# tzt101/MichiGAN

Measured on AMD Instinct MI355X. Metric: training images/sec at 512x512 (G+D step), higher is better.
Workload: dtype bf16; 1 GPU; SPADEB G + multiscale PatchGAN D + VGG19 + Gabor orientation losses, full G step + D step (Adam), bs=8/GPU, 512x512, BASELINE.json configs[2]; global_batch=8, batch_per_gpu=8, resolution=512, parallelism=dp1, init=reference default (xavier, 0.02), random VGG weights

## Files before the change

michigan_amd/csrc/mg_wgrad.hip:

```cpp
#include "mg_common.h"
#include "mg_wgrad_common.h"
#include "mg_options.h"



namespace {

constexpr int NTHR = 256;

struct WgK {
    const void* x; const void* dy; float* dw; float* dbias;
    int N, Hin, Win, Cin, Hj, Wj, Cg, isy, isx, ntaps;
    int K;
    int kper;
    int tiles_m, tiles_n, splitk;
    int tpt;
    long det_stride;
    int tap[MG_MAX_TAPS];
};

template <typename T, bool TR>
__global__ __launch_bounds__(NTHR) void wgrad_kernel(const WgK d)
{
    constexpr bool BF = (sizeof(T) == 2);
    constexpr int KP  = BF ? 32 : 16;
    constexpr int EPP = 16 / (int)sizeof(T);
    constexpr int PPR = 128 * (int)sizeof(T) / 16;
    constexpr int RPP = NTHR / PPR;
    constexpr int NPASS = KP / RPP;
    constexpr int RS  = BF ? 320 : 528;
    constexpr int OPB = KP * RS;
    constexpr int STAGE = 2 * OPB;

    extern __shared__ __attribute__((aligned(16))) unsigned char smem[];

    const int tid = threadIdx.x, lane = tid & 63, wave = tid >> 6;
    const int wm = wave >> 1, wn = wave & 1;
    const int l31 = lane & 31, hi = lane >> 5;

    int tile;
    {
        const int nblk = gridDim.x, b = blockIdx.x;
        const int q8 = nblk >> 3, r8 = nblk & 7, xcd = b & 7, idx = b >> 3;
        tile = (xcd < r8 ? xcd * (q8 + 1) : r8 * (q8 + 1) + (xcd - r8) * q8) + idx;
    }
    const int ngroups = (d.ntaps + d.tpt - 1) / d.tpt;
    const int tm = tile % d.tiles_m;  tile /= d.tiles_m;
    const int tn = tile % d.tiles_n;  tile /= d.tiles_n;
    const int tg = tile % ngroups;
    const int split = tile / ngroups;
    const int m0 = tm * 128, n0 = tn * 128;
    const int tap0 = tg * d.tpt;
    const int kbeg = split * d.kper;
    const int kend = min(d.K, kbeg + d.kper);
    if (kbeg >= kend) return;


    const T* __restrict__ X  = reinterpret_cast<const T*>(d.x);
    const T* __restrict__ DY = reinterpret_cast<const T*>(d.dy);
    const int HWj = d.Hj * d.Wj;

    const int piece = tid % PPR, prow = tid / PPR;
    const int ca = m0 + piece * EPP;
    const bool cav = ca < d.Cg;
    int mytap, cb;
    if (d.tpt > 1) { const int e = piece * EPP; mytap = tap0 + e / d.Cin; cb = e % d.Cin; }
    else           { mytap = tap0; cb = n0 + piece * EPP; }
    const bool cbv = (mytap < d.ntaps) && (cb < d.Cin);
    const int tp = d.tap[mytap < d.ntaps ? mytap : 0];
    const int tdy = (int)(short)(tp & 0xffff), tdx = tp >> 16;

    uint4 ra[NPASS], rb[NPASS];
    auto gload = [&](int k0) {
#pragma unroll
        for (int i = 0; i < NPASS; ++i) {
            const int q = k0 + prow + i * RPP;
            uint4 va = make_uint4(0, 0, 0, 0), vb = make_uint4(0, 0, 0, 0);
            if (q < kend) {
                if (cav) va = *reinterpret_cast<const uint4*>(DY + ((size_t)q * d.Cg + ca));
                if (cbv) {
                    const int n = q / HWj, r = q - n * HWj;
                    const int jy = r / d.Wj, jx = r - jy * d.Wj;
                    const int iy = jy * d.isy + tdy, ix = jx * d.isx + tdx;
                    if ((unsigned)iy < (unsigned)d.Hin && (unsigned)ix < (unsigned)d.Win)
                        vb = *reinterpret_cast<const uint4*>(X + ((size_t)((n * d.Hin + iy) * d.Win + ix) * d.Cin + cb));
                }
            }
            ra[i] = va; rb[i] = vb;
        }
    };
    auto lstore = [&](int s) {
        unsigned char* base = smem + s * STAGE;
#pragma unroll
        for (int i = 0; i < NPASS; ++i) {
            const int row = prow + i * RPP;
            *reinterpret_cast<uint4*>(base + row * RS + piece * 16) = ra[i];
            *reinterpret_cast<uint4*>(base + OPB + row * RS + piece * 16) = rb[i];
        }
    };

    f32x16_t acc[2][2];
#pragma unroll
    for (int mt = 0; mt < 2; ++mt)
#pragma unroll
        for (int nt = 0; nt < 2; ++nt)
#pragma unroll
            for (int r = 0; r < 16; ++r) acc[mt][nt][r] = 0.f;

    const bool do_bias = d.dbias != nullptr && tg == 0 && tn == 0;
    float bsum[EPP];
#pragma unroll
    for (int j = 0; j < EPP; ++j) bsum[j] = 0.f;
    auto bias_acc = [&]() {
#pragma unroll
        for (int i = 0; i < NPASS; ++i) {
            const uint32_t w[4] = {ra[i].x, ra[i].y, ra[i].z, ra[i].w};
            if constexpr (BF) {
#pragma unroll
                for (int j = 0; j < 4; ++j) { bsum[2 * j] += __uint_as_float(w[j] << 16); bsum[2 * j + 1] += __uint_as_float(w[j] & 0xffff0000u); }
            } else {
#pragma unroll
                for (int j = 0; j < 4; ++j) bsum[j] += __uint_as_float(w[j]);
            }
        }
    };

    auto compute = [&](int s) {
        const unsigned char* As = smem + s * STAGE;
        const unsigned char* Bs = As + OPB;
        if constexpr (BF) {
#pragma unroll
            for (int ks = 0; ks < 2; ++ks) {
                bf16x8_t a[2], b[2];
                if constexpr (TR) {
                    const int i16 = lane & 15, g2 = lane >> 4;
                    const int row = ks * 16 + (g2 >> 1) * 8 + (i16 >> 2);
                    const int col = (g2 & 1) * 16 + (i16 & 3) * 4;
#pragma unroll
                    for (int t = 0; t < 2; ++t) {
                        typedef __attribute__((address_space(3))) s16x4_t* lp_t;
                        const unsigned char* pa = As + row * RS + (wm * 64 + t * 32 + col) * 2;
                        const unsigned char* pb = Bs + row * RS + (wn * 64 + t * 32 + col) * 2;
                        s16x4_t a0 = __builtin_amdgcn_ds_read_tr16_b64_v4i16((lp_t)(pa));
                        s16x4_t a1 = __builtin_amdgcn_ds_read_tr16_b64_v4i16((lp_t)(pa + 4 * RS));
                        s16x4_t b0 = __builtin_amdgcn_ds_read_tr16_b64_v4i16((lp_t)(pb));
                        s16x4_t b1 = __builtin_amdgcn_ds_read_tr16_b64_v4i16((lp_t)(pb + 4 * RS));
                        typedef __attribute__((ext_vector_type(8))) short s16x8_t;
                        s16x8_t av = __builtin_shufflevector(a0, a1, 0, 1, 2, 3, 4, 5, 6, 7);
                        s16x8_t bv = __builtin_shufflevector(b0, b1, 0, 1, 2, 3, 4, 5, 6, 7);
                        a[t] = __builtin_bit_cast(bf16x8_t, av);
                        b[t] = __builtin_bit_cast(bf16x8_t, bv);
                    }
                } else {
                    typedef __attribute__((ext_vector_type(8))) short s16x8_t;
#pragma unroll
                    for (int t = 0; t < 2; ++t) {
                        s16x8_t av, bv;
#pragma unroll
                        for (int j = 0; j < 8; ++j) {
                            const int row = ks * 16 + hi * 8 + j;
                            av[j] = *reinterpret_cast<const short*>(As + row * RS + (wm * 64 + t * 32 + l31) * 2);
                            bv[j] = *reinterpret_cast<const short*>(Bs + row * RS + (wn * 64 + t * 32 + l31) * 2);
                        }
                        a[t] = __builtin_bit_cast(bf16x8_t, av);
                        b[t] = __builtin_bit_cast(bf16x8_t, bv);
                    }
                }
#pragma unroll
                for (int mt = 0; mt < 2; ++mt)
#pragma unroll
                    for (int nt = 0; nt < 2; ++nt)
                        acc[mt][nt] = __builtin_amdgcn_mfma_f32_32x32x16_bf16(a[mt], b[nt], acc[mt][nt], 0, 0, 0);
            }
        } else {
            f32x16_t t[2][2];
#pragma unroll
            for (int kk = 0; kk < KP / 2; ++kk) {
                float a[2], b[2];
                const int row = kk * 2 + hi;
#pragma unroll
                for (int q = 0; q < 2; ++q) {
                    a[q] = *reinterpret_cast<const float*>(As + row * RS + (wm * 64 + q * 32 + l31) * 4);
                    b[q] = *reinterpret_cast<const float*>(Bs + row * RS + (wn * 64 + q * 32 + l31) * 4);
                }
#pragma unroll
                for (int mt = 0; mt < 2; ++mt)
#pragma unroll
                    for (int nt = 0; nt < 2; ++nt) {
                        f32x16_t c;
                        if (MG_F32_ONE_CHAIN) {
                            acc[mt][nt] = __builtin_amdgcn_mfma_f32_32x32x2f32(a[mt], b[nt], acc[mt][nt], 0, 0, 0);
                            continue;
                        }
                        if (kk == 0) {
#pragma unroll
                            for (int e = 0; e < 16; ++e) c[e] = 0.f;
                        } else {
                            c = t[mt][nt];
                        }
                        t[mt][nt] = __builtin_amdgcn_mfma_f32_32x32x2f32(a[mt], b[nt], c, 0, 0, 0);
                    }
            }
#pragma unroll
            for (int mt = 0; mt < 2; ++mt)
#pragma unroll
                for (int nt = 0; nt < 2; ++nt) {
                    if (MG_F32_ONE_CHAIN) continue;
                    acc[mt][nt] += t[mt][nt];
                    asm volatile("" : "+v"(acc[mt][nt]));
                }
        }
    };

    const int nk = (kend - kbeg + KP - 1) / KP;
    gload(kbeg);
    if (do_bias) bias_acc();
    lstore(0);
    __syncthreads();
    for (int it = 0; it < nk; ++it) {
        const bool more = (it + 1 < nk);
        if (more) gload(kbeg + (it + 1) * KP);
        compute(it & 1);
        if (more) { if (do_bias) bias_acc(); lstore((it + 1) & 1); }
        __syncthreads();
    }
    if (do_bias) {
        float* red = reinterpret_cast<float*>(smem);
#pragma unroll
        for (int j = 0; j < EPP; ++j) red[prow * 128 + piece * EPP + j] = bsum[j];
        __syncthreads();
        if (tid < 128 && m0 + tid < d.Cg) {
            float t = 0.f;
            for (int r = 0; r < RPP; ++r) t += red[r * 128 + tid];
            wg_accum(d.dbias, d.det_stride, split, (size_t)(m0 + tid), t);
        }
    }

#pragma unroll
    for (int mt = 0; mt < 2; ++mt)
#pragma unroll
        for (int nt = 0; nt < 2; ++nt) {
            const int nn = wn * 64 + nt * 32 + l31;
            int tap, ci;
            if (d.tpt > 1) { tap = tap0 + nn / d.Cin; ci = nn % d.Cin; }
            else           { tap = tap0; ci = n0 + nn; }
            if (tap >= d.ntaps || ci >= d.Cin) continue;
#pragma unroll
            for (int r = 0; r < 16; ++r) {
                const int co = m0 + wm * 64 + mt * 32 + (r & 3) + 8 * (r >> 2) + 4 * hi;
                if (co < d.Cg)
                    wg_accum(d.dw, d.det_stride, split, (size_t)(tap * d.Cg + co) * d.Cin + ci, acc[mt][nt][r]);
            }
        }
}

__global__ __launch_bounds__(256) void wgrad_det_finish_kernel(const float* __restrict__ ws, int nsplit, long stride, float* __restrict__ dw, long ndw,
                                                               float* __restrict__ dbias, int nbias)
{
    __shared__ float red[256];
    const long total = ndw + nbias;
    const int cl = threadIdx.x & 31, row = threadIdx.x >> 5;
    for (long i0 = blockIdx.x * 32L; i0 < total; i0 += gridDim.x * 32L) {
        const long i = i0 + cl;
        float a = 0.f;
        if (i < total) {
            const float* p = ws + i;
            int sp = row;
            for (; sp + 24 < nsplit; sp += 32) {
                const float v0 = p[(size_t)sp * stride], v1 = p[(size_t)(sp + 8) * stride], v2 = p[(size_t)(sp + 16) * stride], v3 = p[(size_t)(sp + 24) * stride];
                a += v0; a += v1; a += v2; a += v3;
            }
            for (; sp < nsplit; sp += 8) a += p[(size_t)sp * stride];
        }
        __syncthreads();
        red[threadIdx.x] = a;
        __syncthreads();
        if (row == 0 && i < total) {
#pragma unroll
            for (int r = 1; r < 8; ++r) a += red[r * 32 + cl];
            if (i < ndw) dw[i] += a; else dbias[i - ndw] += a;
        }
    }
}

template <typename T, bool TR>
int launch_wgrad(WgK& k, hipStream_t st, int* nsplit = nullptr, bool dry = false)
{
    constexpr bool BF = (sizeof(T) == 2);
    constexpr int KP = BF ? 32 : 16;
    constexpr int RS = BF ? 320 : 528;
    k.tiles_m = (k.Cg + 127) / 128;
    k.tpt = (k.Cin < 128 && 128 % k.Cin == 0) ? 128 / k.Cin : 1;
    k.tiles_n = k.tpt > 1 ? 1 : (k.Cin + 127) / 128;
    const long base = (long)k.tiles_m * k.tiles_n * ((k.ntaps + k.tpt - 1) / k.tpt);
    int S = k.splitk;
    if (S <= 0) {
        S = (int)((1536 + base - 1) / base);
        const int min_stages = mg_opt(MG_OPT_WGRAD_MIN_STAGES);
        int maxS = (k.K + KP * min_stages - 1) / (KP * min_stages);
        if (base * maxS < 256) {
            const int fill = (int)((256 + base - 1) / base), floor4 = (k.K + KP * 4 - 1) / (KP * 4);
            maxS = fill < floor4 ? fill : floor4;
        }
        if (S > maxS) S = maxS;
        if (S < 1) S = 1;
    }
    k.kper = ((k.K + S - 1) / S + KP - 1) / KP * KP;
    S = (k.K + k.kper - 1) / k.kper;
    k.splitk = S;
    const long nblk = base * S;
    if (nsplit) *nsplit = S;
    if (dry) return MG_OK;
    if (nblk <= 0 || nblk > 0x7fffffffL) return mg_fail(MG_ERR_ARG, "mg_conv_wgrad: bad grid %ld", nblk);
    const size_t lds = 2 * 2 * (size_t)KP * RS;
    hipLaunchKernelGGL((wgrad_kernel<T, TR>), dim3((unsigned)nblk), dim3(NTHR), lds, st, k);
    MG_CHECK_LAUNCH("mg_conv_wgrad");
    return MG_OK;
}

}

int launch_wgrad_det_finish(const float* ws, int nsplit, long stride, float* dw, long ndw, float* dbias, int nbias, hipStream_t st)
{
    const long total = ndw + nbias;
    long grid = (total + 31) / 32;
    if (grid > 8192) grid = 8192;
    hipLaunchKernelGGL(wgrad_det_finish_kernel, dim3((unsigned)grid), dim3(256), 0, st, ws, nsplit, stride, dw, ndw, dbias, nbias);
    MG_CHECK_LAUNCH("mg_conv_wgrad(deterministic finish)");
    return MG_OK;
}

namespace {

int route_wgrad(const mg_wgrad_desc* d, hipStream_t st, float* dw, float* dbias, long det_stride, int* nsplit, bool dry)
{
    WgK k;
    k.x = d->x; k.dy = d->dy; k.dw = dw; k.dbias = dbias;
    k.N = d->N; k.Hin = d->Hin; k.Win = d->Win; k.Cin = d->Cin;
    k.Hj = d->Hj; k.Wj = d->Wj; k.Cg = d->Cg; k.isy = d->isy; k.isx = d->isx; k.ntaps = d->ntaps;
    k.K = d->N * d->Hj * d->Wj; k.splitk = d->splitk; k.kper = 0; k.tiles_m = k.tiles_n = 0; k.tpt = 1; k.det_stride = det_stride;
    for (int t = 0; t < MG_MAX_TAPS; ++t)
        k.tap[t] = t < d->ntaps ? (int)((((uint32_t)(int)d->tap_dy[t]) & 0xffffu) | (((uint32_t)(int)d->tap_dx[t]) << 16)) : 0;
    if (d->dtype == MG_BF16 && d->ntaps == 9 && d->isy == 1 && d->isx == 1 && d->Hin == d->Hj && d->Win == d->Wj && d->Cin == 8) {
        bool std3x3 = true;
        for (int t = 0; t < 9; ++t) std3x3 = std3x3 && d->tap_dy[t] == t / 3 - 1 && d->tap_dx[t] == t % 3 - 1;
        Wg3K k3;
        k3.x = d->x; k3.dy = d->dy; k3.dw = dw; k3.dbias = dbias;
        k3.N = d->N; k3.H = d->Hin; k3.W = d->Win; k3.Cin = d->Cin; k3.Cg = d->Cg;
        k3.nstg = 0; k3.sps = 0; k3.tiles_m = k3.tiles_n = 0; k3.splitk = 0; k3.det_stride = det_stride; k3.half_cu = 0; k3.stripe_w = 0;
        if (std3x3 && wgrad_thin_applies(k3)) return launch_wgrad_thin(k3, st, nsplit, dry);
    }
    if (wgrad_thin_taps_applies(d)) return launch_wgrad_thin_taps(d, st, dw, dbias, det_stride, nsplit, dry);
    if (mg_opt(MG_OPT_WGRAD3X3) && d->dtype == MG_BF16 && (d->flags & 1) && d->ntaps == 9 && d->isy == 1 && d->isx == 1 &&
        d->Hin == d->Hj && d->Win == d->Wj && (d->Win == 16 || d->Win % 32 == 0) && (d->Hin * d->Win) % 32 == 0 &&
        d->Cin >= 64 && d->Cg >= 64) {
        bool std3x3 = true;
        for (int t = 0; t < 9; ++t) std3x3 = std3x3 && d->tap_dy[t] == t / 3 - 1 && d->tap_dx[t] == t % 3 - 1;
        if (std3x3) {
            Wg3K k3;
            k3.x = d->x; k3.dy = d->dy; k3.dw = dw; k3.dbias = dbias;
            k3.N = d->N; k3.H = d->Hin; k3.W = d->Win; k3.Cin = d->Cin; k3.Cg = d->Cg;
            k3.nstg = k.K / 32; k3.sps = 0; k3.tiles_m = k3.tiles_n = 0; k3.splitk = d->splitk; k3.det_stride = det_stride;
            k3.half_cu = (d->flags & 2) ? 1 : 0; k3.stripe_w = 0;
            return launch_wgrad3x3(k3, st, nsplit, dry);
        }
    }
    if (d->dtype == MG_BF16)
        return (d->flags & 1) ? launch_wgrad<uint16_t, true>(k, st, nsplit, dry) : launch_wgrad<uint16_t, false>(k, st, nsplit, dry);
    return launch_wgrad<float, false>(k, st, nsplit, dry);
}

int check_wgrad_desc(const mg_wgrad_desc* d, const char* who)
{
    MG_CHECK_ARG(d != nullptr, "%s: null descriptor", who);
    MG_CHECK_ARG(d->x && d->dy && d->dw, "%s: null tensor pointer", who);
    MG_CHECK_ARG(d->dtype == MG_F32 || d->dtype == MG_BF16, "%s: bad dtype %d", who, d->dtype);
    MG_CHECK_ARG(d->ntaps >= 1 && d->ntaps <= MG_MAX_TAPS, "%s: ntaps=%d out of range", who, d->ntaps);
    MG_CHECK_ARG(d->Cin > 0 && (d->Cin % 8) == 0 && d->Cg > 0 && (d->Cg % 8) == 0,
                 "%s: Cin=%d / Cg=%d must be positive multiples of 8", who, d->Cin, d->Cg);
    MG_CHECK_ARG(d->N > 0 && d->Hj > 0 && d->Wj > 0 && d->Hin > 0 && d->Win > 0, "%s: empty geometry", who);
    MG_CHECK_ARG((long)d->N * d->Hj * d->Wj < (1L << 30), "%s: too many pixels", who);
    return MG_OK;
}

}

extern "C" int64_t mg_wgrad_det_workspace(const mg_wgrad_desc* d)
{
    if (check_wgrad_desc(d, "mg_wgrad_det_workspace") != MG_OK) return -1;
    int S = 0;
    if (route_wgrad(d, nullptr, d->dw, d->dbias, 0, &S, true) != MG_OK || S <= 0) return -1;
    const long slab = (long)d->ntaps * d->Cg * d->Cin + (d->dbias ? d->Cg : 0);
    return (int64_t)S * slab * (int64_t)sizeof(float);
}

extern "C" int mg_conv_wgrad(const mg_wgrad_desc* d, void* stream)
{
    const int rc = check_wgrad_desc(d, "mg_conv_wgrad");
    if (rc != MG_OK) return rc;
    hipStream_t st = reinterpret_cast<hipStream_t>(stream);
    if (d->det_ws == nullptr) return route_wgrad(d, st, d->dw, d->dbias, 0, nullptr, false);
    int S = 0;
    if (route_wgrad(d, st, d->dw, d->dbias, 0, &S, true) != MG_OK || S <= 0) return mg_fail(MG_ERR_ARG, "mg_conv_wgrad: cannot size the deterministic workspace");
    const long ndw = (long)d->ntaps * d->Cg * d->Cin, nbias = d->dbias ? d->Cg : 0, slab = ndw + nbias;
    MG_CHECK_ARG(d->det_ws_bytes >= (int64_t)S * slab * (int64_t)sizeof(float), "mg_conv_wgrad: deterministic workspace too small (%ld splits)", (long)S);
    float* ws = reinterpret_cast<float*>(d->det_ws);
    int S2 = 0;
    const int r2 = route_wgrad(d, st, ws, d->dbias ? ws + ndw : nullptr, slab, &S2, false);
    if (r2 != MG_OK) return r2;
    if (S2 != S) return mg_fail(MG_ERR_LAUNCH, "mg_conv_wgrad: split count changed between sizing and launch (%d vs %d)", S, S2);
    return launch_wgrad_det_finish(ws, S, slab, d->dw, ndw, d->dbias, (int)nbias, st);
}
```

michigan_amd/csrc/mg_wgrad3x3.hip:

```cpp
#include "mg_conv_common.h"
#include "mg_wgrad_common.h"


namespace {

typedef __attribute__((ext_vector_type(4))) short s16x4_t;
typedef __attribute__((ext_vector_type(8))) short s16x8_t;
typedef __attribute__((address_space(3))) s16x4_t* lds_s16x4_p;

__device__ unsigned long long* g_mg_wg3_probe_out = nullptr;
__device__ __forceinline__ unsigned long long wg3_stamp()
{
    unsigned long long v;
    asm volatile("s_memrealtime %0\n\ts_waitcnt lgkmcnt(0)" : "=s"(v) :: "memory");
    return v;
}

template <int MT, int NT, bool W16, bool PROBE = false>
__global__ __launch_bounds__(256, 2) void wgrad3x3_kernel(const Wg3K d)
{
    constexpr int TM = 64 * MT, TN = 64 * NT;
    constexpr int RBA = TM * 2, RBB = TN * 2;
    constexpr int PPA = RBA / 16, PPB = RBB / 16;
    constexpr int A_ROWS = 32, B_ROWS = (NT == 2) ? 36 : 40;
    constexpr int A_BYTES = A_ROWS * RBA, B_BYTES = B_ROWS * RBB;
    constexpr int A_IPS = A_BYTES / 4096;
    constexpr int B_IPS = (B_BYTES + 4095) / 4096;
    constexpr int IPS = A_IPS + B_IPS;
    constexpr int STAGE = A_BYTES + B_BYTES;
    constexpr int NS = 4;
    static_assert(A_BYTES % 4096 == 0 && B_BYTES % 1024 == 0, "stage must be whole wave blocks");

    extern __shared__ __attribute__((aligned(16))) unsigned char smem[];

    const int tid = threadIdx.x, lane = tid & 63;
    const int wave = __builtin_amdgcn_readfirstlane(tid >> 6);
    const int wm = wave >> 1, wn = wave & 1;
    const int l31 = lane & 31, hi = lane >> 5;

    int tile;
    {
        const int nblk = gridDim.x, b = blockIdx.x;
        const int q8 = nblk >> 3, r8 = nblk & 7, xcd = b & 7, idx = b >> 3;
        tile = (xcd < r8 ? xcd * (q8 + 1) : r8 * (q8 + 1) + (xcd - r8) * q8) + idx;
    }
    const int tm = tile % d.tiles_m;  tile /= d.tiles_m;
    const int tn = tile % d.tiles_n;  tile /= d.tiles_n;
    const int ky = tile % 3;
    const int split = tile / 3;
    const int m0 = tm * TM, n0 = tn * TN;
    const int sbeg = split * d.sps;
    const int send = min(d.nstg, sbeg + d.sps);
    const int nk = send - sbeg;
    if (nk <= 0) return;

    const int H = d.H, W = d.W;
    constexpr int SEG = W16 ? 16 : 32, SEGP = SEG + 2;
    constexpr int PR = (32 / SEG) * SEGP;
    const unsigned lds0 = (unsigned)(size_t)(__attribute__((address_space(3))) unsigned char*)smem;
    const unsigned dump = lds0 + NS * STAGE + wave * 1024;
    const unsigned char* zsrc = g_mg_zeros + (lane & 3) * 16;

    auto swz_a = [](int row) { return RBA == 256 ? (row & 3) : ((row >> 1) & 1); };
    auto swz_b = [](int row) { return RBB == 256 ? (row & 3) : ((row >> 1) & 1); };

    int aoff[A_IPS];
#pragma unroll
    for (int j = 0; j < A_IPS; ++j) {
        const int g = j * 256 + tid, row = g / PPA, slot = g % PPA;
        int ch = m0 + ((slot ^ (swz_a(row) << 2)) << 3);
        if (ch >= d.Cg) ch = m0;
        aoff[j] = (row * d.Cg + ch) * 2;
    }
    int boff[B_IPS], brc[B_IPS];
#pragma unroll
    for (int j = 0; j < B_IPS; ++j) {
        const int g = j * 256 + tid, row = g / PPB, slot = g % PPB;
        int ch = n0 + ((slot ^ (swz_b(row) << 2)) << 3);
        if (ch >= d.Cin) ch = n0;
        const int r = (W16 && row >= SEGP) ? 1 : 0, c = row - r * SEGP - 1;
        boff[j] = (((r + ky - 1) * W + c) * d.Cin + ch) * 2;
        brc[j] = row < PR ? (r | (c + 1) << 4) : -1;
    }
    const unsigned char* const dy0 = reinterpret_cast<const unsigned char*>(d.dy);
    const unsigned char* const x0p = reinterpret_cast<const unsigned char*>(d.x);
    const unsigned char* abase; const unsigned char* xbase;
    int sy, sx, sg_next = sbeg;
    int simg = 0, sstripe = 0;
    const int SWp = W16 ? W : d.stripe_w, nsegs = SWp / 32, nstripes = W / SWp;
    if (W16) {
        abase = dy0 + (size_t)sbeg * 32 * d.Cg * 2;
        xbase = x0p + (size_t)sbeg * 32 * d.Cin * 2;
        const int rem = (sbeg * 32) % (H * W); sy = rem / W; sx = rem - sy * W;
    } else {
        const int spi = H * (W / 32);
        simg = sbeg / spi;
        int r = sbeg - simg * spi;
        sstripe = r / (H * nsegs);  r -= sstripe * (H * nsegs);
        sy = r / nsegs;
        sx = sstripe * SWp + (r - sy * nsegs) * 32;
        const size_t p = ((size_t)simg * H + sy) * W + sx;
        abase = dy0 + p * d.Cg * 2;
        xbase = x0p + p * d.Cin * 2;
    }
    sy = __builtin_amdgcn_readfirstlane(sy); sx = __builtin_amdgcn_readfirstlane(sx);
    simg = __builtin_amdgcn_readfirstlane(simg); sstripe = __builtin_amdgcn_readfirstlane(sstripe);
    const int a_step = 32 * d.Cg * 2, x_step = 32 * d.Cin * 2;

    unsigned long long m_live[B_IPS], m_left[B_IPS], m_right[B_IPS], m_r1[B_IPS];
#pragma unroll
    for (int j = 0; j < B_IPS; ++j) {
        const bool lv = brc[j] >= 0;
        const int c = (brc[j] >> 4) - 1, r = brc[j] & 15;
        m_live[j]  = __builtin_amdgcn_ballot_w64(lv);
        m_left[j]  = __builtin_amdgcn_ballot_w64(lv && c == -1);
        m_right[j] = __builtin_amdgcn_ballot_w64(lv && c == SEG);
        m_r1[j]    = __builtin_amdgcn_ballot_w64(lv && r == 1);
    }
    const unsigned long long zaddr = (unsigned long long)(size_t)zsrc;
    const unsigned zlo = (unsigned)zaddr, zhi = (unsigned)(zaddr >> 32);

    auto issue = [&](int stage) {
        const bool real = sg_next < send;
        const unsigned sbase = lds0 + stage * STAGE;
        if (real) {
#pragma unroll
            for (int j = 0; j < A_IPS; ++j)
                glds16_s(abase, (unsigned)aoff[j], __builtin_amdgcn_readfirstlane(sbase + j * 4096 + wave * 1024));
        } else {
#pragma unroll
            for (int j = 0; j < A_IPS; ++j)
                glds16(zsrc, __builtin_amdgcn_readfirstlane(sbase + j * 4096 + wave * 1024));
        }
        const int sxs = __builtin_amdgcn_readfirstlane(sx), sys = __builtin_amdgcn_readfirstlane(sy), kys = __builtin_amdgcn_readfirstlane(ky);
        const bool lok = sxs > 0, rok = sxs + SEG < W;
        const bool y0 = (unsigned)(sys + kys - 1) < (unsigned)H, y1 = (unsigned)(sys + kys) < (unsigned)H;
#pragma unroll
        for (int j = 0; j < B_IPS; ++j) {
            unsigned long long v = real ? m_live[j] : 0ull;
            if (!lok) v &= ~m_left[j];
            if (!rok) v &= ~m_right[j];
            if (W16) { if (!y0) v &= m_r1[j]; if (!y1) v &= ~m_r1[j]; }
            else if (!y0) v = 0ull;
            v = ((unsigned long long)(unsigned)__builtin_amdgcn_readfirstlane((int)(v >> 32)) << 32) | (unsigned)__builtin_amdgcn_readfirstlane((int)v);
            asm("" : "+s"(v));
            const unsigned long long pa = (unsigned long long)(size_t)(xbase + boff[j]);
            unsigned plo, phi;
            asm("v_cndmask_b32_e64 %0, %1, %2, %3" : "=v"(plo) : "v"(zlo), "v"((unsigned)pa), "s"(v));
            asm("v_cndmask_b32_e64 %0, %1, %2, %3" : "=v"(phi) : "v"(zhi), "v"((unsigned)(pa >> 32)), "s"(v));
            const bool live = (j * 4096 + wave * 1024) < B_BYTES;
            glds16(reinterpret_cast<const void*>((size_t)(((unsigned long long)phi << 32) | plo)),
                   __builtin_amdgcn_readfirstlane(live ? sbase + A_BYTES + j * 4096 + wave * 1024 : dump));
        }
        ++sg_next;
        if (W16) {
            abase += a_step; xbase += x_step;
            sy += 2; if (sy >= H) sy = 0;
        } else {
            sx += 32;
            if (sx < (sstripe + 1) * SWp) { abase += a_step; xbase += x_step; }
            else {
                sx = sstripe * SWp; ++sy;
                if (sy >= H) { sy = 0; ++sstripe; if (sstripe >= nstripes) { sstripe = 0; ++simg; } sx = sstripe * SWp; }
                const size_t p = ((size_t)simg * H + sy) * W + sx;
                abase = dy0 + p * d.Cg * 2;
                xbase = x0p + p * d.Cin * 2;
            }
        }
    };

    f32x16_t acc[3][MT][NT];
#pragma unroll
    for (int kx = 0; kx < 3; ++kx)
#pragma unroll
        for (int mt = 0; mt < MT; ++mt)
#pragma unroll
            for (int nt = 0; nt < NT; ++nt)
#pragma unroll
                for (int r = 0; r < 16; ++r) acc[kx][mt][nt][r] = 0.f;

    const bool do_bias = d.dbias != nullptr && ky == 1 && tn == 0 && wn == 0;
    float bsum[MT];
#pragma unroll
    for (int mt = 0; mt < MT; ++mt) bsum[mt] = 0.f;

    const int i16 = lane & 15, g2 = lane >> 4;
    const int rsub = (g2 >> 1) * 8 + (i16 >> 2);
    const int csub = ((g2 & 1) * 16 + (i16 & 3) * 4) * 2;
    constexpr int ksb = W16 ? SEGP : 16;

    auto compute = [&](int slot) {
        const unsigned char* As = smem + slot * STAGE;
        const unsigned char* Bs = As + A_BYTES;
#pragma unroll
        for (int ks = 0; ks < 2; ++ks) {
            bf16x8_t a[MT];
            const int ra = ks * 16 + rsub;
#pragma unroll
            for (int mt = 0; mt < MT; ++mt) {
                const int col = ((wm * MT + mt) * 64 + csub) ^ (swz_a(ra) << 6);
                const unsigned char* p = As + ra * RBA + col;
                s16x4_t v0 = __builtin_amdgcn_ds_read_tr16_b64_v4i16((lds_s16x4_p)(p));
                s16x4_t v1 = __builtin_amdgcn_ds_read_tr16_b64_v4i16((lds_s16x4_p)(p + 4 * RBA));
                a[mt] = __builtin_bit_cast(bf16x8_t, __builtin_shufflevector(v0, v1, 0, 1, 2, 3, 4, 5, 6, 7));
                if (do_bias) {
                    typedef __attribute__((ext_vector_type(4))) unsigned u32x4_t;
                    const u32x4_t w = __builtin_bit_cast(u32x4_t, a[mt]);
#pragma unroll
                    for (int j = 0; j < 4; ++j) bsum[mt] += __uint_as_float(w[j] << 16) + __uint_as_float(w[j] & 0xffff0000u);
                }
            }
            static_for<0, 3>([&](auto kx_) {
                constexpr int kx = decltype(kx_)::value;
                bf16x8_t b[NT];
                const int rb = ks * ksb + kx + rsub;
#pragma unroll
                for (int nt = 0; nt < NT; ++nt) {
                    const int col = ((wn * NT + nt) * 64 + csub) ^ (swz_b(rb) << 6);
                    const unsigned char* p = Bs + rb * RBB + col;
                    s16x4_t v0 = __builtin_amdgcn_ds_read_tr16_b64_v4i16((lds_s16x4_p)(p));
                    s16x4_t v1 = __builtin_amdgcn_ds_read_tr16_b64_v4i16((lds_s16x4_p)(p + 4 * RBB));
                    b[nt] = __builtin_bit_cast(bf16x8_t, __builtin_shufflevector(v0, v1, 0, 1, 2, 3, 4, 5, 6, 7));
                }
#pragma unroll
                for (int mt = 0; mt < MT; ++mt)
#pragma unroll
                    for (int nt = 0; nt < NT; ++nt)
                        acc[kx][mt][nt] = __builtin_amdgcn_mfma_f32_32x32x16_bf16(a[mt], b[nt], acc[kx][mt][nt], 0, 0, 0);
            });
        }
    };

#pragma unroll
    for (int s = 0; s < NS - 1; ++s) issue(s);
    int slot = 0, islot = NS - 1;
    unsigned long long t_wait = 0, t_bar = 0, t_issue = 0, t_mfma = 0, t_begin = 0;
    if constexpr (PROBE) t_begin = wg3_stamp();
    for (int it = 0; it < nk; ++it) {
        unsigned long long s0 = 0, s1 = 0, s2 = 0, s3 = 0;
        if constexpr (PROBE) s0 = wg3_stamp();
        wait_vmcnt<(NS - 2) * IPS>();
        if constexpr (PROBE) s1 = wg3_stamp();
        __builtin_amdgcn_s_barrier();
        if constexpr (PROBE) s2 = wg3_stamp();
        issue(islot);
        if constexpr (PROBE) s3 = wg3_stamp();
        compute(slot);
        if constexpr (PROBE) { const unsigned long long s4 = wg3_stamp(); t_wait += s1 - s0; t_bar += s2 - s1; t_issue += s3 - s2; t_mfma += s4 - s3; }
        slot = (slot == NS - 1) ? 0 : slot + 1;
        islot = (islot == NS - 1) ? 0 : islot + 1;
    }
    wait_vmcnt<0>();
    unsigned long long t_loop_end = 0;
    if constexpr (PROBE) t_loop_end = wg3_stamp();

    if (do_bias) {
#pragma unroll
        for (int mt = 0; mt < MT; ++mt) {
            const float t = bsum[mt] + __shfl_xor(bsum[mt], 32);
            const int co = m0 + (wm * MT + mt) * 32 + l31;
            if (hi == 0 && co < d.Cg) wg_accum(d.dbias, d.det_stride, split, (size_t)co, t);
        }
    }

    static_for<0, 3 * MT * NT>([&](auto i_) {
        constexpr int kx = decltype(i_)::value / (MT * NT), mt = (decltype(i_)::value / NT) % MT, nt = decltype(i_)::value % NT;
        const int ci = n0 + (wn * NT + nt) * 32 + l31;
        if (ci >= d.Cin) return;
        const int tap = ky * 3 + kx;
#pragma unroll
        for (int r = 0; r < 16; ++r) {
            const int co = m0 + (wm * MT + mt) * 32 + (r & 3) + 8 * (r >> 2) + 4 * hi;
            if (co < d.Cg)
                wg_accum(d.dw, d.det_stride, split, (size_t)(tap * d.Cg + co) * d.Cin + ci, acc[kx][mt][nt][r]);
        }
    });
    if constexpr (PROBE) {
        const unsigned long long t_end = wg3_stamp();
        if (lane == 0 && g_mg_wg3_probe_out) {
            unsigned long long* o = g_mg_wg3_probe_out + ((size_t)blockIdx.x * 4 + wave) * 8;
            o[0] = t_wait; o[1] = t_bar; o[2] = t_issue; o[3] = t_mfma; o[4] = t_loop_end - t_begin; o[5] = t_end - t_loop_end; o[6] = (unsigned long long)nk; o[7] = t_begin;
        }
    }
}


template <int MT, int NT, bool W16>
int launch3(Wg3K& k, hipStream_t st, int* nsplit, bool dry)
{
    constexpr int TM = 64 * MT, TN = 64 * NT;
    constexpr int STAGE = 32 * TM * 2 + ((NT == 2) ? 36 : 40) * TN * 2;
    constexpr size_t LDS = 4 * (size_t)STAGE + 4096;
    k.tiles_m = (k.Cg + TM - 1) / TM;
    k.tiles_n = (k.Cin + TN - 1) / TN;
    const int stripe = mg_opt(MG_OPT_WGRAD3X3_STRIPE);
    k.stripe_w = (!W16 && stripe >= 32 && (stripe % 32) == 0 && k.W > stripe && (k.W % stripe) == 0) ? stripe : k.W;
    const long base = 3L * k.tiles_m * k.tiles_n;
    int S = k.splitk;
    if (S <= 0) {
        const int lo = (int)((384 + base - 1) / base), hi = (int)((1536 + base - 1) / base);
        S = k.nstg / 192 < hi ? k.nstg / 192 : hi;
        if (S < lo) S = lo;
        if (S > k.nstg / 16) S = k.nstg / 16;
        if (S < 1) S = 1;
    }
    if (S > k.nstg) S = k.nstg;
    k.sps = (k.nstg + S - 1) / S;
    S = (k.nstg + k.sps - 1) / k.sps;
    const long nblk = base * S;
    if (nsplit) *nsplit = S;
    if (dry) return MG_OK;
    if (nblk <= 0 || nblk > 0x7fffffffL) return mg_fail(MG_ERR_ARG, "mg_conv_wgrad: bad grid %ld", nblk);
    auto kern = wgrad3x3_kernel<MT, NT, W16>;
    constexpr size_t LDS_HALF_CU = LDS > 84 * 1024 ? LDS : 84 * 1024;
    const size_t lds_req = k.half_cu ? LDS_HALF_CU : LDS;
    mg_raise_lds_cap(reinterpret_cast<const void*>(kern), (int)LDS_HALF_CU);
#if MG_PROBES
    if constexpr (MT == 2 && NT == 2 && !W16) {
        if (mg_opt(MG_OPT_PROBE_WGRAD3X3)) {
            auto pk = wgrad3x3_kernel<MT, NT, W16, true>;
            mg_raise_lds_cap(reinterpret_cast<const void*>(pk), (int)LDS);
            hipLaunchKernelGGL(pk, dim3((unsigned)nblk), dim3(256), LDS, st, k);
            MG_CHECK_LAUNCH("mg_conv_wgrad(3x3 probe)");
            return MG_OK;
        }
    }
#endif
    hipLaunchKernelGGL(kern, dim3((unsigned)nblk), dim3(256), lds_req, st, k);
    MG_CHECK_LAUNCH("mg_conv_wgrad(3x3)");
    return MG_OK;
}

}

int wgrad3x3_set_probe(unsigned long long addr)
{
    unsigned long long* p = reinterpret_cast<unsigned long long*>(addr);
    return hipMemcpyToSymbol(HIP_SYMBOL(g_mg_wg3_probe_out), &p, sizeof(p)) == hipSuccess ? MG_OK : MG_ERR_ARG;
}

int launch_wgrad3x3(Wg3K& k, hipStream_t st, int* nsplit, bool dry)
{
    const bool m2 = k.Cg > 64, n2 = k.Cin > 64;
    if (k.W == 16) {
        if (m2 && n2) return launch3<2, 2, true>(k, st, nsplit, dry);
        if (m2)       return launch3<2, 1, true>(k, st, nsplit, dry);
        if (n2)       return launch3<1, 2, true>(k, st, nsplit, dry);
        return launch3<1, 1, true>(k, st, nsplit, dry);
    }
    if (m2 && n2) return launch3<2, 2, false>(k, st, nsplit, dry);
    if (m2)       return launch3<2, 1, false>(k, st, nsplit, dry);
    if (n2)       return launch3<1, 2, false>(k, st, nsplit, dry);
    return launch3<1, 1, false>(k, st, nsplit, dry);
}
```

michigan_amd/csrc/mg_wgrad_common.h:

```cpp
#pragma once
#include "mg_common.h"

struct Wg3K {
    const void* x; const void* dy; float* dw; float* dbias;
    int N, H, W, Cin, Cg;
    int nstg;
    int sps;
    int tiles_m, tiles_n;
    int splitk;
    long det_stride;
    int half_cu;
    int stripe_w;
};

__device__ __forceinline__ void wg_accum(float* base, long det_stride, int split, size_t idx, float v)
{
    if (det_stride) base[(size_t)split * det_stride + idx] = v;
    else atomicAdd(base + idx, v);
}
int launch_wgrad_det_finish(const float* ws, int nsplit, long stride, float* dw, long ndw, float* dbias, int nbias, hipStream_t st);

int launch_wgrad3x3(Wg3K& k, hipStream_t st, int* nsplit = nullptr, bool dry = false);
bool wgrad_thin_applies(const Wg3K& k);
int launch_wgrad_thin(Wg3K& k, hipStream_t st, int* nsplit = nullptr, bool dry = false);

struct WgT {
    const void* x; const void* dy; float* ws;
    int N, Hin, Win, Hj, Wj, ntaps;
    int HH, HW, dy0, dx0;
    long slab;
    int has_bias;
    int tap[MG_MAX_TAPS];
};
bool wgrad_thin_taps_applies(const mg_wgrad_desc* d);
int launch_wgrad_thin_taps(const mg_wgrad_desc* d, hipStream_t st, float* dw, float* dbias, long det_stride, int* nsplit, bool dry);
float* mg_stream_scratch(hipStream_t st, size_t bytes);
```

Before: 131.5 images/s.

## Plan wgrad split-K with occupancy-aware cost model and balanced splits

Replaces the fixed split-K heuristics in the generic and 3x3 weight-gradient launchers with a cost model. It queries resident block slots per CU and picks a split count that trades wave rounds against atomic flush traffic. Splits now use a quotient/remainder range so stage counts are balanced across blocks. The atomic flush order is also rotated per split so concurrent blocks hit different output rows first, which should reduce atomic contention. Risks are mis-tuned cost constants and extra host-side occupancy queries, though those are cached.

```diff
diff --git a/michigan_amd/csrc/mg_wgrad.hip b/michigan_amd/csrc/mg_wgrad.hip
--- a/michigan_amd/csrc/mg_wgrad.hip
+++ b/michigan_amd/csrc/mg_wgrad.hip
@@ -12,7 +12,7 @@
     const void* x; const void* dy; float* dw; float* dbias;
     int N, Hin, Win, Cin, Hj, Wj, Cg, isy, isx, ntaps;
     int K;
-    int kper;
+    int sq, sr;
     int tiles_m, tiles_n, splitk;
     int tpt;
     long det_stride;
@@ -51,8 +51,10 @@
     const int split = tile / ngroups;
     const int m0 = tm * 128, n0 = tn * 128;
     const int tap0 = tg * d.tpt;
-    const int kbeg = split * d.kper;
-    const int kend = min(d.K, kbeg + d.kper);
+    int s0, s1;
+    wg_split_range(d.sq, d.sr, split, s0, s1);
+    const int kbeg = s0 * KP;
+    const int kend = min(d.K, s1 * KP);
     if (kbeg >= kend) return;
 
 
@@ -236,10 +238,14 @@
         }
     }
 
+    const int rot = __builtin_amdgcn_readfirstlane(split & 3);
+#pragma unroll
+    for (int pass = 0; pass < 2; ++pass)
 #pragma unroll
     for (int mt = 0; mt < 2; ++mt)
 #pragma unroll
         for (int nt = 0; nt < 2; ++nt) {
+            if ((mt * 2 + nt >= rot) != (pass == 0)) continue;
             const int nn = wn * 64 + nt * 32 + l31;
             int tap, ci;
             if (d.tpt > 1) { tap = tap0 + nn / d.Cin; ci = nn % d.Cin; }
@@ -283,6 +289,8 @@
     }
 }
 
+constexpr WgCost WG_COST_PER_CU = {0.364f, 0.f, 2.05e6f};
+
 template <typename T, bool TR>
 int launch_wgrad(WgK& k, hipStream_t st, int* nsplit = nullptr, bool dry = false)
 {
@@ -293,26 +301,26 @@
     k.tpt = (k.Cin < 128 && 128 % k.Cin == 0) ? 128 / k.Cin : 1;
     k.tiles_n = k.tpt > 1 ? 1 : (k.Cin + 127) / 128;
     const long base = (long)k.tiles_m * k.tiles_n * ((k.ntaps + k.tpt - 1) / k.tpt);
-    int S = k.splitk;
-    if (S <= 0) {
-        S = (int)((1536 + base - 1) / base);
-        const int min_stages = mg_opt(MG_OPT_WGRAD_MIN_STAGES);
-        int maxS = (k.K + KP * min_stages - 1) / (KP * min_stages);
-        if (base * maxS < 256) {
-            const int fill = (int)((256 + base - 1) / base), floor4 = (k.K + KP * 4 - 1) / (KP * 4);
-            maxS = fill < floor4 ? fill : floor4;
-        }
-        if (S > maxS) S = maxS;
-        if (S < 1) S = 1;
-    }
-    k.kper = ((k.K + S - 1) / S + KP - 1) / KP * KP;
-    S = (k.K + k.kper - 1) / k.kper;
+    const size_t lds = 2 * 2 * (size_t)KP * RS;
+    const int nstg = (k.K + KP - 1) / KP;
+    const int min_stages = mg_opt(MG_OPT_WGRAD_MIN_STAGES);
+    int maxS = (nstg + min_stages - 1) / min_stages;
+    if (base * maxS < 256) {
+        const int fill = (int)((256 + base - 1) / base), floor4 = (nstg + 3) / 4;
+        maxS = fill < floor4 ? fill : floor4;
+    }
+    int per = 2;
+    const int slots = wg_resident_slots(reinterpret_cast<const void*>(&wgrad_kernel<T, TR>), NTHR, lds, 2, &per);
+    WgCost cost = WG_COST_PER_CU;
+    cost.stage_us *= (float)per * (BF ? 1.f : 4.f);
+    const WgPlan plan = wg_plan_split(base, nstg, slots, 128L * 128 * 4, maxS, k.splitk, cost);
+    const int S = plan.S;
+    k.sq = plan.q; k.sr = plan.r;
     k.splitk = S;
-    const long nblk = base * S;
+    const long nblk = plan.nblk;
     if (nsplit) *nsplit = S;
     if (dry) return MG_OK;
     if (nblk <= 0 || nblk > 0x7fffffffL) return mg_fail(MG_ERR_ARG, "mg_conv_wgrad: bad grid %ld", nblk);
-    const size_t lds = 2 * 2 * (size_t)KP * RS;
     hipLaunchKernelGGL((wgrad_kernel<T, TR>), dim3((unsigned)nblk), dim3(NTHR), lds, st, k);
     MG_CHECK_LAUNCH("mg_conv_wgrad");
     return MG_OK;
@@ -338,7 +346,7 @@
     k.x = d->x; k.dy = d->dy; k.dw = dw; k.dbias = dbias;
     k.N = d->N; k.Hin = d->Hin; k.Win = d->Win; k.Cin = d->Cin;
     k.Hj = d->Hj; k.Wj = d->Wj; k.Cg = d->Cg; k.isy = d->isy; k.isx = d->isx; k.ntaps = d->ntaps;
-    k.K = d->N * d->Hj * d->Wj; k.splitk = d->splitk; k.kper = 0; k.tiles_m = k.tiles_n = 0; k.tpt = 1; k.det_stride = det_stride;
+    k.K = d->N * d->Hj * d->Wj; k.splitk = d->splitk; k.sq = k.sr = 0; k.tiles_m = k.tiles_n = 0; k.tpt = 1; k.det_stride = det_stride;
     for (int t = 0; t < MG_MAX_TAPS; ++t)
         k.tap[t] = t < d->ntaps ? (int)((((uint32_t)(int)d->tap_dy[t]) & 0xffffu) | (((uint32_t)(int)d->tap_dx[t]) << 16)) : 0;
     if (d->dtype == MG_BF16 && d->ntaps == 9 && d->isy == 1 && d->isx == 1 && d->Hin == d->Hj && d->Win == d->Wj && d->Cin == 8) {
@@ -347,7 +355,7 @@
         Wg3K k3;
         k3.x = d->x; k3.dy = d->dy; k3.dw = dw; k3.dbias = dbias;
         k3.N = d->N; k3.H = d->Hin; k3.W = d->Win; k3.Cin = d->Cin; k3.Cg = d->Cg;
-        k3.nstg = 0; k3.sps = 0; k3.tiles_m = k3.tiles_n = 0; k3.splitk = 0; k3.det_stride = det_stride; k3.half_cu = 0; k3.stripe_w = 0;
+        k3.nstg = 0; k3.sps = k3.srem = 0; k3.tiles_m = k3.tiles_n = 0; k3.splitk = 0; k3.det_stride = det_stride; k3.half_cu = 0; k3.stripe_w = 0;
         if (std3x3 && wgrad_thin_applies(k3)) return launch_wgrad_thin(k3, st, nsplit, dry);
     }
     if (wgrad_thin_taps_applies(d)) return launch_wgrad_thin_taps(d, st, dw, dbias, det_stride, nsplit, dry);
@@ -360,7 +368,7 @@
             Wg3K k3;
             k3.x = d->x; k3.dy = d->dy; k3.dw = dw; k3.dbias = dbias;
             k3.N = d->N; k3.H = d->Hin; k3.W = d->Win; k3.Cin = d->Cin; k3.Cg = d->Cg;
-            k3.nstg = k.K / 32; k3.sps = 0; k3.tiles_m = k3.tiles_n = 0; k3.splitk = d->splitk; k3.det_stride = det_stride;
+            k3.nstg = k.K / 32; k3.sps = k3.srem = 0; k3.tiles_m = k3.tiles_n = 0; k3.splitk = d->splitk; k3.det_stride = det_stride;
             k3.half_cu = (d->flags & 2) ? 1 : 0; k3.stripe_w = 0;
             return launch_wgrad3x3(k3, st, nsplit, dry);
         }
diff --git a/michigan_amd/csrc/mg_wgrad3x3.hip b/michigan_amd/csrc/mg_wgrad3x3.hip
--- a/michigan_amd/csrc/mg_wgrad3x3.hip
+++ b/michigan_amd/csrc/mg_wgrad3x3.hip
@@ -49,8 +49,9 @@
     const int ky = tile % 3;
     const int split = tile / 3;
     const int m0 = tm * TM, n0 = tn * TN;
-    const int sbeg = split * d.sps;
-    const int send = min(d.nstg, sbeg + d.sps);
+    int sbeg, send;
+    wg_split_range(d.sps, d.srem, split, sbeg, send);
+    send = min(send, d.nstg);
     const int nk = send - sbeg;
     if (nk <= 0) return;
 
@@ -263,7 +264,9 @@
         }
     }
 
-    static_for<0, 3 * MT * NT>([&](auto i_) {
+    constexpr int NBLK = 3 * MT * NT;
+    const int rot = __builtin_amdgcn_readfirstlane(split % NBLK);
+    auto flush = [&](auto i_) {
         constexpr int kx = decltype(i_)::value / (MT * NT), mt = (decltype(i_)::value / NT) % MT, nt = decltype(i_)::value % NT;
         const int ci = n0 + (wn * NT + nt) * 32 + l31;
         if (ci >= d.Cin) return;
@@ -274,7 +277,9 @@
             if (co < d.Cg)
                 wg_accum(d.dw, d.det_stride, split, (size_t)(tap * d.Cg + co) * d.Cin + ci, acc[kx][mt][nt][r]);
         }
-    });
+    };
+    static_for<0, NBLK>([&](auto i_) { if (decltype(i_)::value >= rot) flush(i_); });
+    static_for<0, NBLK>([&](auto i_) { if (decltype(i_)::value < rot) flush(i_); });
     if constexpr (PROBE) {
         const unsigned long long t_end = wg3_stamp();
         if (lane == 0 && g_mg_wg3_probe_out) {
@@ -284,6 +289,9 @@
     }
 }
 
+
+constexpr WgCost WG3_COST_ONE_PER_CU = {0.864f, 1.5f, 1.65e6f};
+constexpr WgCost WG3_COST_TWO_PER_CU = {1.189f, 0.f, 1.62e6f};
 
 template <int MT, int NT, bool W16>
 int launch3(Wg3K& k, hipStream_t st, int* nsplit, bool dry)
@@ -296,25 +304,20 @@
     const int stripe = mg_opt(MG_OPT_WGRAD3X3_STRIPE);
     k.stripe_w = (!W16 && stripe >= 32 && (stripe % 32) == 0 && k.W > stripe && (k.W % stripe) == 0) ? stripe : k.W;
     const long base = 3L * k.tiles_m * k.tiles_n;
-    int S = k.splitk;
-    if (S <= 0) {
-        const int lo = (int)((384 + base - 1) / base), hi = (int)((1536 + base - 1) / base);
-        S = k.nstg / 192 < hi ? k.nstg / 192 : hi;
-        if (S < lo) S = lo;
-        if (S > k.nstg / 16) S = k.nstg / 16;
-        if (S < 1) S = 1;
-    }
-    if (S > k.nstg) S = k.nstg;
-    k.sps = (k.nstg + S - 1) / S;
-    S = (k.nstg + k.sps - 1) / k.sps;
-    const long nblk = base * S;
-    if (nsplit) *nsplit = S;
-    if (dry) return MG_OK;
-    if (nblk <= 0 || nblk > 0x7fffffffL) return mg_fail(MG_ERR_ARG, "mg_conv_wgrad: bad grid %ld", nblk);
     auto kern = wgrad3x3_kernel<MT, NT, W16>;
     constexpr size_t LDS_HALF_CU = LDS > 84 * 1024 ? LDS : 84 * 1024;
     const size_t lds_req = k.half_cu ? LDS_HALF_CU : LDS;
     mg_raise_lds_cap(reinterpret_cast<const void*>(kern), (int)LDS_HALF_CU);
+    const int slots = wg_resident_slots(reinterpret_cast<const void*>(kern), 256, lds_req, k.half_cu ? 1 : 2);
+    WgCost cost = k.half_cu ? WG3_COST_ONE_PER_CU : WG3_COST_TWO_PER_CU;
+    cost.stage_us *= (float)(MT * NT) / 4.f;
+    const WgPlan plan = wg_plan_split(base, k.nstg, slots, 3L * TM * TN * 4, k.nstg / 16, k.splitk, cost);
+    const int S = plan.S;
+    k.sps = plan.q; k.srem = plan.r;
+    const long nblk = plan.nblk;
+    if (nsplit) *nsplit = S;
+    if (dry) return MG_OK;
+    if (nblk <= 0 || nblk > 0x7fffffffL) return mg_fail(MG_ERR_ARG, "mg_conv_wgrad: bad grid %ld", nblk);
 #if MG_PROBES
     if constexpr (MT == 2 && NT == 2 && !W16) {
         if (mg_opt(MG_OPT_PROBE_WGRAD3X3)) {
diff --git a/michigan_amd/csrc/mg_wgrad_common.h b/michigan_amd/csrc/mg_wgrad_common.h
--- a/michigan_amd/csrc/mg_wgrad_common.h
+++ b/michigan_amd/csrc/mg_wgrad_common.h
@@ -1,11 +1,91 @@
 #pragma once
+
+struct WgCost {
+    float stage_us;
+    float fixed_us;
+    float atomic_bpus;
+};
+struct WgPlan {
+    int S;
+    int q, r;
+    long nblk;
+    int rounds;
+};
+
+#if defined(__HIPCC__)
+#define MG_PLAN_HD __host__ __device__
+#else
+#define MG_PLAN_HD
+#endif
+MG_PLAN_HD static inline void wg_split_range(int q, int r, int split, int& beg, int& end)
+{
+    beg = split * q + (split < r ? split : r);
+    end = beg + q + (split < r ? 1 : 0);
+}
+
+static inline float wg_plan_cost(long base, int nstg, int slots, long flush_bytes, int S, const WgCost& c)
+{
+    const long nblk = base * S, rounds = (nblk + slots - 1) / slots;
+    return (float)rounds * ((float)((nstg + S - 1) / S) * c.stage_us + c.fixed_us) + (float)nblk * (float)flush_bytes / c.atomic_bpus;
+}
+
+static inline WgPlan wg_plan_split(long base, int nstg, int slots, long flush_bytes, int max_split, int splitk, const WgCost& c)
+{
+    if (base < 1) base = 1;
+    if (nstg < 1) nstg = 1;
+    if (slots < 1) slots = 1;
+    int S = splitk;
+    if (S <= 0) {
+        if (max_split > nstg) max_split = nstg;
+        if (max_split < 1) max_split = 1;
+        const bool whole = base <= slots;
+        float best = 0.f;
+        long prev = 0;
+        for (int i = 1; i <= 8 && prev < max_split; ++i) {
+            long cand = whole ? (long)i * slots / base : i;
+            if (cand > max_split) cand = max_split;
+            if (cand <= prev) continue;
+            const float t = wg_plan_cost(base, nstg, slots, flush_bytes, (int)cand, c);
+            if (prev == 0 || t < best) { best = t; S = (int)cand; }
+            prev = cand;
+        }
+    }
+    if (S > nstg) S = nstg;
+    WgPlan p;
+    p.S = S; p.q = nstg / S; p.r = nstg % S;
+    p.nblk = base * S;
+    p.rounds = (int)((p.nblk + slots - 1) / slots);
+    return p;
+}
+
+#ifndef MG_WGRAD_PLAN_ONLY
 #include "mg_common.h"
+
+static inline int wg_resident_slots(const void* kern, int threads, size_t lds, int fallback_per_cu, int* per_cu = nullptr)
+{
+    static std::mutex mu;
+    static struct { const void* k; int dev; size_t lds; int cus, per; } seen[64];
+    static int nseen = 0;
+    int dev = 0;
+    (void)hipGetDevice(&dev);
+    std::lock_guard<std::mutex> lock(mu);
+    int cus = 0, per = 0;
+    for (int i = 0; i < nseen && !per; ++i)
+        if (seen[i].k == kern && seen[i].dev == dev && seen[i].lds == lds) { cus = seen[i].cus; per = seen[i].per; }
+    if (!per) {
+        if (hipDeviceGetAttribute(&cus, hipDeviceAttributeMultiprocessorCount, dev) != hipSuccess || cus <= 0) { (void)hipGetLastError(); cus = 256; }
+        if (hipOccupancyMaxActiveBlocksPerMultiprocessor(&per, kern, threads, lds) != hipSuccess || per <= 0) { (void)hipGetLastError(); per = fallback_per_cu; }
+        if (nseen < 64) { seen[nseen].k = kern; seen[nseen].dev = dev; seen[nseen].lds = lds; seen[nseen].cus = cus; seen[nseen].per = per; ++nseen; }
+    }
+    if (per_cu) *per_cu = per;
+    return cus * per;
+}
 
 struct Wg3K {
     const void* x; const void* dy; float* dw; float* dbias;
     int N, H, W, Cin, Cg;
     int nstg;
-    int sps;
+    int sps, srem;
     int tiles_m, tiles_n;
     int splitk;
     long det_stride;
@@ -35,3 +115,4 @@
 bool wgrad_thin_taps_applies(const mg_wgrad_desc* d);
 int launch_wgrad_thin_taps(const mg_wgrad_desc* d, hipStream_t st, float* dw, float* dbias, long det_stride, int* nsplit, bool dry);
 float* mg_stream_scratch(hipStream_t st, size_t bytes);
+#endif
```

New measurement: 130.0 images/s. -1.1%, worse.
